# playHing/Scaled-MMD-GAN

Measured on AMD Instinct MI355X. Metric: images/sec/step (64x64 SMMD, batch 64) + MMD-kernel GB/s at 1/2/4/8 GPU, higher is better.
Workload: dtype fp32; 1 GPU; imagenet_smmd 64x64 SNResNet G/D, rbf kernel, scaling, SN, batch 64/GPU, 5D+1G schedule; model=snresnet, global_batch=64, parallelism=dp1, dp_mode=global, dp_forced=False, memory_format=nchw, miopen_winograd=True, miopen_find=False, step_graphs=False, conv_mean_pool=folded 4x4 stride-2 conv, miopen_db=/tmp/code/home/pair/home_parent/tmp/smmd_miopen_db_fofa0w5q

## Files before the change

scaled-mmd-gan_amd/csrc/smmd_wino_s2_wgrad.hip:

```cpp
#include "smmd_wino_common.hpp"

namespace smmd {

namespace {

constexpr int W2_T = 512;
struct for_wino4x4s2_wgrad {};

template <int CT, int RT>
struct S2w {
    static constexpr int NI = 16 / (CT * RT);
    static constexpr int TPI = CT * RT;
    static constexpr int XR = 4 * RT + 2;
    static constexpr int XRS = 4 * CT + 2;
    static constexpr int XS = ((NI * XR * XRS + 3) & ~7) + 4;
    static constexpr int GRS = 2 * CT;
    static constexpr int GS = (NI * 2 * RT * 2 * CT) | 1;
    static constexpr int STAGE = 16 * XS + 64 * GS;
    static constexpr size_t LDS = 2 * STAGE * sizeof(float);
    static constexpr int XF4 = 16 * NI * XR * CT;
    static constexpr int GF4 = 64 * NI * (TPI);
    static constexpr int NX = (XF4 + W2_T - 1) / W2_T;
    static constexpr int NG = (GF4 + W2_T - 1) / W2_T;
    static_assert(CT * RT * NI == 16, "16 tiles per chunk");
    static_assert(XS >= NI * XR * XRS && XS % 8 == 4, "x channel stride");
    static_assert(XRS % 4 == 2, "x row stride");
    static_assert(LDS >= 4 * 9 * 8 * 64 * sizeof(float), "epilogue hand-off fits");
    static_assert(LDS <= 160 * 1024, "LDS budget");
};

struct S2wGeom {
    int N, C, K, H, W;
    int TH, TW, Timg;
    int64_t T;
    int chunks_per_slice;
};

template <int CT, int RT>
__global__ __launch_bounds__(W2_T, 1) void s2_wgrad_kernel(
    const float *__restrict__ x, const float *__restrict__ gy, float *__restrict__ part,
    S2wGeom g) {
    using P = S2w<CT, RT>;
    extern __shared__ float4 s2w_lds4[];
    float *const lds = reinterpret_cast<float *>(s2w_lds4);

    const int tid = threadIdx.x, lane = tid & 63, w = tid >> 6;
    const int kb = blockIdx.x, cb = blockIdx.y, sl = blockIdx.z;
    const int HW = g.H * g.W, Ho = g.H / 2, Wo = g.W / 2, HWo = Ho * Wo;
    const int64_t nchunks_all = g.T / 16;
    const int64_t ch0 = (int64_t)sl * g.chunks_per_slice;
    const int nchunk = (int)min((int64_t)g.chunks_per_slice, nchunks_all - ch0);
    const int cpi = g.Timg >= 16 ? g.Timg / 16 : 1;

    float4 xr[P::NX], gr[P::NG];
    auto gload = [&](int64_t chunk) {
        int n0, ty0;
        if (P::NI > 1) {
            n0 = (int)(chunk * P::NI);
            ty0 = 0;
        } else {
            const uint32_t ch32 = (uint32_t)chunk;
            n0 = (int)(ch32 / (uint32_t)cpi);
            ty0 = (int)(ch32 - (uint32_t)n0 * (uint32_t)cpi) * RT;
        }
        const uint32_t xrange = (uint32_t)(((P::NI - 1) * g.C + 16) * HW) * 4u;
        const uint32_t grange = (uint32_t)(((P::NI - 1) * g.K + 64) * HWo) * 4u;
        const __amdgpu_buffer_rsrc_t xs = __builtin_amdgcn_make_buffer_rsrc(
            const_cast<float *>(x + ((int64_t)n0 * g.C + cb * 16) * HW), 0, xrange, 0x00020000);
        const __amdgpu_buffer_rsrc_t gs = __builtin_amdgcn_make_buffer_rsrc(
            const_cast<float *>(gy + ((int64_t)n0 * g.K + kb * 64) * HWo), 0, grange, 0x00020000);
#pragma unroll
        for (int i = 0; i < P::NX; ++i) {
            const int idx = min(i * W2_T + tid, P::XF4 - 1);
            const int f = idx % CT, rr = idx / CT;
            const int r = rr % P::XR, ci = rr / P::XR;
            const int c = ci % 16, img = ci / 16;
            const int yy = 4 * ty0 - 1 + r;
            const uint32_t off = (yy >= 0 && yy < g.H)
                                     ? (uint32_t)((img * g.C + c) * HW + yy * g.W + 4 * f) * 4u
                                     : BUF_OOB;
            xr[i] = __builtin_bit_cast(float4, __builtin_amdgcn_raw_buffer_load_b128(xs, off, 0, 0));
        }
#pragma unroll
        for (int i = 0; i < P::NG; ++i) {
            const int idx = min(i * W2_T + tid, P::GF4 - 1);
            const int f = idx % P::TPI, ki = idx / P::TPI;
            const int k = ki % 64, img = ki / 64;
            const uint32_t off =
                (uint32_t)((img * g.K + k) * HWo + (2 * ty0) * Wo + 4 * f) * 4u;
            gr[i] = __builtin_bit_cast(float4, __builtin_amdgcn_raw_buffer_load_b128(gs, off, 0, 0));
        }
    };
    auto lstore = [&](int buf) {
        float *X = lds + buf * P::STAGE;
        float *Gd = X + 16 * P::XS;
#pragma unroll
        for (int i = 0; i < P::NX; ++i) {
            const int idx = min(i * W2_T + tid, P::XF4 - 1);
            const int f = idx % CT, rr = idx / CT;
            const int r = rr % P::XR, ci = rr / P::XR;
            const int c = ci % 16, img = ci / 16;
            float *d = X + c * P::XS + (img * P::XR + r) * P::XRS + 1 + 4 * f;
            d[0] = xr[i].x; d[1] = xr[i].y; d[2] = xr[i].z; d[3] = xr[i].w;
        }
#pragma unroll
        for (int i = 0; i < P::NG; ++i) {
            const int idx = min(i * W2_T + tid, P::GF4 - 1);
            const int f = idx % P::TPI, ki = idx / P::TPI;
            const int k = ki % 64, img = ki / 64;
            float *d = Gd + k * P::GS + img * (4 * P::TPI) + 4 * f;
            d[0] = gr[i].x; d[1] = gr[i].y; d[2] = gr[i].z; d[3] = gr[i].w;
        }
    };

    const int tp = w >> 2, kh = (w >> 1) & 1, ch = w & 1, hl = lane >> 5, l32 = lane & 31;
    const int cp = ch * 32 + l32;
    const int cl = cp >> 2, pi = (cp >> 1) & 1, pj = cp & 1;
    auto lds_read = [&](int buf, int s, float (&d)[9], float (&gv)[4]) {
        const float *X = lds + buf * P::STAGE;
        const float *Gd = X + 16 * P::XS;
        const int tau = 2 * s + hl;
        const int img = tau / P::TPI, loc = tau % P::TPI;
        const int ty = loc / CT, tx = loc % CT;
        const float *xc = X + cl * P::XS + (img * P::XR + 4 * ty + pi) * P::XRS + 4 * tx + pj;
#pragma unroll
        for (int a = 0; a < 3; ++a)
#pragma unroll
            for (int b = 0; b < 3; ++b) d[a * 3 + b] = xc[(2 * a) * P::XRS + 2 * b];
        const float *gk = Gd + (kh * 32 + l32) * P::GS + img * (4 * P::TPI) + (2 * ty) * P::GRS +
                          2 * tx;
        gv[0] = gk[0]; gv[1] = gk[1]; gv[2] = gk[P::GRS]; gv[3] = gk[P::GRS + 1];
    };
    auto tslice = [&](int q, const float (&d)[9], const float (&gv)[4], float (&t)[9],
                      float (&a)[9], float (&b)[9]) {
        if (q == 1) {
            const float r0[2] = {gv[0], gv[1]};
            const float r1[2] = {gv[0] + gv[2], gv[1] + gv[3]};
            const float r2[2] = {gv[2], gv[3]};
            a[0] = r0[0]; a[1] = r0[0] + r0[1]; a[2] = r0[1];
            a[3] = r1[0]; a[4] = r1[0] + r1[1]; a[5] = r1[1];
            a[6] = r2[0]; a[7] = r2[0] + r2[1]; a[8] = r2[1];
        } else if (q == 2) {
#pragma unroll
            for (int j = 0; j < 3; ++j) {
                t[j] = d[j] - d[3 + j];
                t[3 + j] = d[3 + j];
                t[6 + j] = d[6 + j] - d[3 + j];
            }
        } else if (q == 3) {
#pragma unroll
            for (int i = 0; i < 3; ++i) {
                b[i * 3 + 0] = t[i * 3 + 0] - t[i * 3 + 1];
                b[i * 3 + 1] = t[i * 3 + 1];
                b[i * 3 + 2] = t[i * 3 + 2] - t[i * 3 + 1];
            }
        }
    };

    f32x16 acc[9];
#pragma unroll
    for (int p = 0; p < 9; ++p) acc[p] = f32x16{};

    for (int i = tid; i < 2 * 16 * P::NI * P::XR; i += W2_T) {
        const int buf = i / (16 * P::NI * P::XR), rc = i % (16 * P::NI * P::XR);
        const int c = rc / (P::NI * P::XR), row = rc % (P::NI * P::XR);
        float *X = lds + buf * P::STAGE + c * P::XS + row * P::XRS;
        X[0] = 0.f;
        X[4 * CT + 1] = 0.f;
    }
    if (nchunk > 0) {
        gload(ch0);
        lstore(0);
        __syncthreads();
        float oa[2][9], ob[2][9];
        {
            float d[9], gv[4], t[9];
            lds_read(0, tp, d, gv);
#pragma unroll
            for (int q = 0; q < 9; ++q) tslice(q, d, gv, t, oa[0], ob[0]);
        }
        for (int c = 0; c < nchunk; ++c) {
            const int buf = c & 1;
            gload(ch0 + min(c + 1, nchunk - 1));
#pragma unroll
            for (int m = 0; m < 4; ++m) {
                const int cur = m & 1, nxt = cur ^ 1;
                float d[9], gv[4], t[9];
                if (m == 3) {
                    lstore(buf ^ 1);
                    __syncthreads();
                }
                __builtin_amdgcn_sched_barrier(0);
                lds_read(m < 3 ? buf : buf ^ 1, m < 3 ? 2 * (m + 1) + tp : tp, d, gv);
                __builtin_amdgcn_sched_barrier(0);
#pragma unroll
                for (int q = 0; q < 9; ++q) {
                    acc[q] = __builtin_amdgcn_mfma_f32_32x32x2f32(oa[cur][q], ob[cur][q], acc[q],
                                                                  0, 0, 0);
                    tslice(q, d, gv, t, oa[nxt], ob[nxt]);
                    __builtin_amdgcn_sched_barrier(0);
                }
            }
        }
    }

    __syncthreads();
    float *out = part + (int64_t)sl * g.K * g.C * 16;
    const int c = cb * 16 + cl;
    float *E = lds + (w & 3) * (9 * 8 * 64);
#pragma unroll
    for (int rh = 0; rh < 2; ++rh) {
        if (tp == 1) {
#pragma unroll
            for (int p = 0; p < 9; ++p)
#pragma unroll
                for (int rr = 0; rr < 8; ++rr) E[(p * 8 + rr) * 64 + lane] = acc[p][rh * 8 + rr];
        }
        __syncthreads();
        if (tp == 0) {
#pragma unroll
            for (int rr = 0; rr < 8; ++rr) {
                const int r = rh * 8 + rr;
                const int k = kb * 64 + kh * 32 + (r & 3) + 8 * (r >> 2) + 4 * hl;
                float u[9];
#pragma unroll
                for (int p = 0; p < 9; ++p) u[p] = acc[p][r] + E[(p * 8 + rr) * 64 + lane];
                float tt[2][3];
#pragma unroll
                for (int j = 0; j < 3; ++j) {
                    tt[0][j] = u[j] + u[3 + j];
                    tt[1][j] = u[3 + j] + u[6 + j];
                }
                float *o = out + ((int64_t)k * g.C + c) * 16;
#pragma unroll
                for (int a = 0; a < 2; ++a) {
                    o[(2 * a + pi) * 4 + pj] = tt[a][0] + tt[a][1];
                    o[(2 * a + pi) * 4 + 2 + pj] = tt[a][1] + tt[a][2];
                }
            }
        }
        __syncthreads();
    }
}

int s2w_shape(int TH, int TW, int *rt) {
    if (TW == 16) { *rt = 1; return 16; }
    if (TW == 8 && TH % 2 == 0) { *rt = 2; return 8; }
    if (TW == 4 && TH % 4 == 0) { *rt = 4; return 4; }
    if (TW == 2 && TH == 2) { *rt = 2; return 2; }
    return 0;
}

template <int CT, int RT>
smmd_status s2w_launch(const float *x, const float *gy, float *part, const S2wGeom &g, int S,
                       hipStream_t st) {
    static bool attr = false;
    if (!attr) {
        if (hipFuncSetAttribute(reinterpret_cast<const void *>(s2_wgrad_kernel<CT, RT>),
                                hipFuncAttributeMaxDynamicSharedMemorySize,
                                (int)S2w<CT, RT>::LDS) != hipSuccess)
            return SMMD_EHIP;
        attr = true;
    }
    s2_wgrad_kernel<CT, RT><<<dim3((unsigned)(g.K / 64), (unsigned)(g.C / 16), (unsigned)S),
                              dim3(W2_T), S2w<CT, RT>::LDS, st>>>(x, gy, part, g);
    return last_launch_status();
}

}

}

using namespace smmd;

extern "C" int smmd_wino4x4s2_wgrad_supported(int n, int ci, int co, int h, int w_img) {
    int rt = 0;
    return n > 0 && ci > 0 && co > 0 && ci % 16 == 0 && co % 64 == 0 && h > 0 && w_img > 0 &&
           h % 4 == 0 && w_img % 4 == 0 && s2w_shape(h / 4, w_img / 4, &rt) != 0 &&
           (int64_t)n * (h / 4) * (w_img / 4) % 16 == 0 &&
           (int64_t)4 * ci * h * w_img * 4 < (1ll << 31) &&
           (int64_t)4 * co * h * w_img < (1ll << 31) && (int64_t)n * (ci + co) * h * w_img < (1ll << 40);
}

extern "C" size_t smmd_wino4x4s2_wgrad_workspace_bytes(int n, int ci, int co, int h, int w_img) {
    if (!smmd_wino4x4s2_wgrad_supported(n, ci, co, h, w_img)) return 0;
    const int64_t T = (int64_t)n * (h / 4) * (w_img / 4);
    const int S = slab_slices((co / 64) * (ci / 16), T / 16, 4);
    return (size_t)(S + slab_groups(S)) * co * ci * 16 * sizeof(float);
}

static smmd_status s2w_launch_all(const float *x, const float *gy, float *gw, int n, int ci,
                                  int co, int h, int w_img, void *ws, size_t ws_bytes, int acc,
                                  smmd_stream_t stream) {
    if (n < 0 || ci <= 0 || co <= 0 || h < 0 || w_img < 0 || !gw) return SMMD_EINVAL;
    hipStream_t st = reinterpret_cast<hipStream_t>(stream);
    if (n == 0 || h == 0 || w_img == 0)
        return acc ? SMMD_OK
                   : hip_status(hipMemsetAsync(gw, 0, (size_t)co * ci * 16 * sizeof(float), st));
    if (!x || !gy) return SMMD_EINVAL;
    if (!smmd_wino4x4s2_wgrad_supported(n, ci, co, h, w_img)) return SMMD_EUNSUPPORTED;
    if ((reinterpret_cast<uintptr_t>(x) | reinterpret_cast<uintptr_t>(gy) |
         reinterpret_cast<uintptr_t>(gw)) & 15)
        return SMMD_EINVAL;
    if (!ws || ws_bytes < smmd_wino4x4s2_wgrad_workspace_bytes(n, ci, co, h, w_img))
        return SMMD_EWORKSPACE;
    if (reinterpret_cast<uintptr_t>(ws) & 15) return SMMD_EINVAL;
    S2wGeom g{};
    g.N = n; g.C = ci; g.K = co; g.H = h; g.W = w_img;
    g.TH = h / 4; g.TW = w_img / 4;
    g.Timg = g.TH * g.TW;
    g.T = (int64_t)n * g.Timg;
    int rt = 0;
    const int ct = s2w_shape(g.TH, g.TW, &rt);
    const int blocks = (co / 64) * (ci / 16);
    const int64_t nchunks = g.T / 16;
    const int S = slab_slices(blocks, nchunks, 4);
    g.chunks_per_slice = (int)((nchunks + S - 1) / S);
    const int Sused = (int)((nchunks + g.chunks_per_slice - 1) / g.chunks_per_slice);
    float *part = static_cast<float *>(ws);
    smmd_status e = ct == 16 ? s2w_launch<16, 1>(x, gy, part, g, Sused, st)
                    : ct == 8 ? s2w_launch<8, 2>(x, gy, part, g, Sused, st)
                    : ct == 4 ? s2w_launch<4, 4>(x, gy, part, g, Sused, st)
                              : s2w_launch<2, 2>(x, gy, part, g, Sused, st);
    if (e != SMMD_OK) return e;
    return slab_sum<for_wino4x4s2_wgrad>(part, Sused, S, (int64_t)co * ci * 4, gw, acc, st);
}

extern "C" smmd_status smmd_wino4x4s2_wgrad(const float *x, const float *gy, float *gw, int n,
                                            int ci, int co, int h, int w_img, void *ws,
                                            size_t ws_bytes, smmd_stream_t stream) {
    return s2w_launch_all(x, gy, gw, n, ci, co, h, w_img, ws, ws_bytes, 0, stream);
}

extern "C" smmd_status smmd_wino4x4s2_wgrad_acc(const float *x, const float *gy, float *gw,
                                                int n, int ci, int co, int h, int w_img,
                                                void *ws, size_t ws_bytes,
                                                smmd_stream_t stream) {
    return s2w_launch_all(x, gy, gw, n, ci, co, h, w_img, ws, ws_bytes, 1, stream);
}
```

Before: 6733 images/s.

## Widen s2 Winograd wgrad block to 32 channels with row-split wave groups

The stride-2 Winograd weight-gradient kernel now covers 32 input channels per block instead of 16. The eight waves are split into two groups that each handle half of the transformed rows (5 or 4 products instead of 9), and the two halves are combined in the epilogue through LDS. Global-to-LDS staging is split into two halves spread across an 8-step inner loop to overlap loads with MFMA, and gy is stored and read as 8-byte pairs. The aim is more reuse of each gy tile per block, fewer redundant transform ops, and better load/compute overlap, at the cost of a larger LDS footprint and half as many blocks along the channel dimension.

```diff
diff --git a/scaled-mmd-gan_amd/csrc/smmd_wino_s2_wgrad.hip b/scaled-mmd-gan_amd/csrc/smmd_wino_s2_wgrad.hip
--- a/scaled-mmd-gan_amd/csrc/smmd_wino_s2_wgrad.hip
+++ b/scaled-mmd-gan_amd/csrc/smmd_wino_s2_wgrad.hip
@@ -15,17 +15,20 @@
     static constexpr int XRS = 4 * CT + 2;
     static constexpr int XS = ((NI * XR * XRS + 3) & ~7) + 4;
     static constexpr int GRS = 2 * CT;
-    static constexpr int GS = (NI * 2 * RT * 2 * CT) | 1;
-    static constexpr int STAGE = 16 * XS + 64 * GS;
+    static constexpr int GS = NI * 2 * RT * 2 * CT + 2;
+    static constexpr int STAGE = 32 * XS + 64 * GS;
     static constexpr size_t LDS = 2 * STAGE * sizeof(float);
-    static constexpr int XF4 = 16 * NI * XR * CT;
-    static constexpr int GF4 = 64 * NI * (TPI);
-    static constexpr int NX = (XF4 + W2_T - 1) / W2_T;
-    static constexpr int NG = (GF4 + W2_T - 1) / W2_T;
-    static_assert(CT * RT * NI == 16, "16 tiles per chunk");
+    static constexpr int XQ = NI * XR * CT;
+    static constexpr int GQ = NI * TPI;
+    static constexpr int NX = (XQ + 15) / 16;
+    static constexpr int NG = GQ / 8;
+    static constexpr int NP = NX + NG;
+    static constexpr int NH = (NP + 1) / 2;
+    static_assert(CT * RT * NI == 16 && 16 % CT == 0 && GQ % 8 == 0, "16 tiles per chunk");
     static_assert(XS >= NI * XR * XRS && XS % 8 == 4, "x channel stride");
     static_assert(XRS % 4 == 2, "x row stride");
-    static_assert(LDS >= 4 * 9 * 8 * 64 * sizeof(float), "epilogue hand-off fits");
+    static_assert(GS % 4 == 2 && GRS % 2 == 0 && STAGE % 2 == 0, "gy pairs 8-byte aligned");
+    static_assert(LDS >= 4 * 2 * 3 * 16 * 64 * sizeof(float), "epilogue hand-off fits");
     static_assert(LDS <= 160 * 1024, "LDS budget");
 };
 
@@ -36,24 +39,29 @@
     int chunks_per_slice;
 };
 
-template <int CT, int RT>
-__global__ __launch_bounds__(W2_T, 1) void s2_wgrad_kernel(
-    const float *__restrict__ x, const float *__restrict__ gy, float *__restrict__ part,
-    S2wGeom g) {
+template <int CT, int RT, int PG>
+__device__ __forceinline__ void s2w_group(const float *__restrict__ x,
+                                          const float *__restrict__ gy,
+                                          float *__restrict__ part, const S2wGeom &g,
+                                          float *const lds, const int cq) {
     using P = S2w<CT, RT>;
-    extern __shared__ float4 s2w_lds4[];
-    float *const lds = reinterpret_cast<float *>(s2w_lds4);
-
-    const int tid = threadIdx.x, lane = tid & 63, w = tid >> 6;
+    constexpr int NPT = PG == 0 ? 5 : 4;
+    const int tid = threadIdx.x, lane = tid & 63;
     const int kb = blockIdx.x, cb = blockIdx.y, sl = blockIdx.z;
     const int HW = g.H * g.W, Ho = g.H / 2, Wo = g.W / 2, HWo = Ho * Wo;
     const int64_t nchunks_all = g.T / 16;
     const int64_t ch0 = (int64_t)sl * g.chunks_per_slice;
     const int nchunk = (int)min((int64_t)g.chunks_per_slice, nchunks_all - ch0);
     const int cpi = g.Timg >= 16 ? g.Timg / 16 : 1;
-
-    float4 xr[P::NX], gr[P::NG];
-    auto gload = [&](int64_t chunk) {
+    const int cw = min(32, g.C - cb * 32);
+
+    const int xc = tid >> 4, xj = tid & 15, gk = tid >> 3, gj = tid & 7;
+    float4 st[P::NP];
+    auto xrow = [&](int i) {
+        const int row = (16 / CT) * i + xj / CT;
+        return 16 * (i + 1) > P::XQ ? min(row, P::NI * P::XR - 1) : row;
+    };
+    auto stage_load = [&](int p0, int p1, int64_t chunk) {
         int n0, ty0;
         if (P::NI > 1) {
             n0 = (int)(chunk * P::NI);
@@ -63,184 +71,200 @@
             n0 = (int)(ch32 / (uint32_t)cpi);
             ty0 = (int)(ch32 - (uint32_t)n0 * (uint32_t)cpi) * RT;
         }
-        const uint32_t xrange = (uint32_t)(((P::NI - 1) * g.C + 16) * HW) * 4u;
+        const uint32_t xrange = (uint32_t)(((P::NI - 1) * g.C + cw) * HW) * 4u;
         const uint32_t grange = (uint32_t)(((P::NI - 1) * g.K + 64) * HWo) * 4u;
         const __amdgpu_buffer_rsrc_t xs = __builtin_amdgcn_make_buffer_rsrc(
-            const_cast<float *>(x + ((int64_t)n0 * g.C + cb * 16) * HW), 0, xrange, 0x00020000);
+            const_cast<float *>(x + ((int64_t)n0 * g.C + cb * 32) * HW), 0, xrange, 0x00020000);
         const __amdgpu_buffer_rsrc_t gs = __builtin_amdgcn_make_buffer_rsrc(
             const_cast<float *>(gy + ((int64_t)n0 * g.K + kb * 64) * HWo), 0, grange, 0x00020000);
 #pragma unroll
         for (int i = 0; i < P::NX; ++i) {
-            const int idx = min(i * W2_T + tid, P::XF4 - 1);
-            const int f = idx % CT, rr = idx / CT;
-            const int r = rr % P::XR, ci = rr / P::XR;
-            const int c = ci % 16, img = ci / 16;
+            if (i < p0 || i >= p1) continue;
+            const int row = xrow(i), f = xj % CT;
+            const int img = P::NI > 1 ? row / P::XR : 0, r = row - img * P::XR;
             const int yy = 4 * ty0 - 1 + r;
             const uint32_t off = (yy >= 0 && yy < g.H)
-                                     ? (uint32_t)((img * g.C + c) * HW + yy * g.W + 4 * f) * 4u
+                                     ? (uint32_t)((img * g.C + xc) * HW + yy * g.W + 4 * f) * 4u
                                      : BUF_OOB;
-            xr[i] = __builtin_bit_cast(float4, __builtin_amdgcn_raw_buffer_load_b128(xs, off, 0, 0));
+            st[i] = __builtin_bit_cast(float4, __builtin_amdgcn_raw_buffer_load_b128(xs, off, 0, 0));
         }
 #pragma unroll
         for (int i = 0; i < P::NG; ++i) {
-            const int idx = min(i * W2_T + tid, P::GF4 - 1);
-            const int f = idx % P::TPI, ki = idx / P::TPI;
-            const int k = ki % 64, img = ki / 64;
+            if (P::NX + i < p0 || P::NX + i >= p1) continue;
+            const int q = gj + 8 * i;
+            const int img = q / P::TPI, f = q % P::TPI;
             const uint32_t off =
-                (uint32_t)((img * g.K + k) * HWo + (2 * ty0) * Wo + 4 * f) * 4u;
-            gr[i] = __builtin_bit_cast(float4, __builtin_amdgcn_raw_buffer_load_b128(gs, off, 0, 0));
-        }
-    };
-    auto lstore = [&](int buf) {
+                (uint32_t)((img * g.K + gk) * HWo + (2 * ty0) * Wo + 4 * f) * 4u;
+            st[P::NX + i] =
+                __builtin_bit_cast(float4, __builtin_amdgcn_raw_buffer_load_b128(gs, off, 0, 0));
+        }
+    };
+    auto stage_store = [&](int p0, int p1, int buf) {
         float *X = lds + buf * P::STAGE;
-        float *Gd = X + 16 * P::XS;
+        float *Gd = X + 32 * P::XS;
 #pragma unroll
         for (int i = 0; i < P::NX; ++i) {
-            const int idx = min(i * W2_T + tid, P::XF4 - 1);
-            const int f = idx % CT, rr = idx / CT;
-            const int r = rr % P::XR, ci = rr / P::XR;
-            const int c = ci % 16, img = ci / 16;
-            float *d = X + c * P::XS + (img * P::XR + r) * P::XRS + 1 + 4 * f;
-            d[0] = xr[i].x; d[1] = xr[i].y; d[2] = xr[i].z; d[3] = xr[i].w;
+            if (i < p0 || i >= p1) continue;
+            float *d = X + xc * P::XS + xrow(i) * P::XRS + 1 + 4 * (xj % CT);
+            d[0] = st[i].x; d[1] = st[i].y; d[2] = st[i].z; d[3] = st[i].w;
         }
 #pragma unroll
         for (int i = 0; i < P::NG; ++i) {
-            const int idx = min(i * W2_T + tid, P::GF4 - 1);
-            const int f = idx % P::TPI, ki = idx / P::TPI;
-            const int k = ki % 64, img = ki / 64;
-            float *d = Gd + k * P::GS + img * (4 * P::TPI) + 4 * f;
-            d[0] = gr[i].x; d[1] = gr[i].y; d[2] = gr[i].z; d[3] = gr[i].w;
-        }
-    };
-
-    const int tp = w >> 2, kh = (w >> 1) & 1, ch = w & 1, hl = lane >> 5, l32 = lane & 31;
-    const int cp = ch * 32 + l32;
+            if (P::NX + i < p0 || P::NX + i >= p1) continue;
+            f2v *d = reinterpret_cast<f2v *>(Gd + gk * P::GS + 4 * (gj + 8 * i));
+            d[0] = f2v{st[P::NX + i].x, st[P::NX + i].y};
+            d[1] = f2v{st[P::NX + i].z, st[P::NX + i].w};
+        }
+    };
+
+    const int hl = lane >> 5, l32 = lane & 31;
+    const int cp = cq * 32 + l32;
     const int cl = cp >> 2, pi = (cp >> 1) & 1, pj = cp & 1;
-    auto lds_read = [&](int buf, int s, float (&d)[9], float (&gv)[4]) {
-        const float *X = lds + buf * P::STAGE;
-        const float *Gd = X + 16 * P::XS;
-        const int tau = 2 * s + hl;
-        const int img = tau / P::TPI, loc = tau % P::TPI;
+    const int xlane = cl * P::XS + (pi + 2 * PG) * P::XRS + pj + 4 * hl;
+    const int glane = 32 * P::XS + l32 * P::GS + 2 * hl;
+    auto lds_read = [&](int buf, int s, float (&d)[6], f2v (&gq)[2][2]) {
+        const int img = (2 * s) / P::TPI, loc = (2 * s) % P::TPI;
         const int ty = loc / CT, tx = loc % CT;
-        const float *xc = X + cl * P::XS + (img * P::XR + 4 * ty + pi) * P::XRS + 4 * tx + pj;
-#pragma unroll
-        for (int a = 0; a < 3; ++a)
-#pragma unroll
-            for (int b = 0; b < 3; ++b) d[a * 3 + b] = xc[(2 * a) * P::XRS + 2 * b];
-        const float *gk = Gd + (kh * 32 + l32) * P::GS + img * (4 * P::TPI) + (2 * ty) * P::GRS +
-                          2 * tx;
-        gv[0] = gk[0]; gv[1] = gk[1]; gv[2] = gk[P::GRS]; gv[3] = gk[P::GRS + 1];
-    };
-    auto tslice = [&](int q, const float (&d)[9], const float (&gv)[4], float (&t)[9],
-                      float (&a)[9], float (&b)[9]) {
-        if (q == 1) {
-            const float r0[2] = {gv[0], gv[1]};
-            const float r1[2] = {gv[0] + gv[2], gv[1] + gv[3]};
-            const float r2[2] = {gv[2], gv[3]};
-            a[0] = r0[0]; a[1] = r0[0] + r0[1]; a[2] = r0[1];
-            a[3] = r1[0]; a[4] = r1[0] + r1[1]; a[5] = r1[1];
-            a[6] = r2[0]; a[7] = r2[0] + r2[1]; a[8] = r2[1];
-        } else if (q == 2) {
-#pragma unroll
-            for (int j = 0; j < 3; ++j) {
-                t[j] = d[j] - d[3 + j];
-                t[3 + j] = d[3 + j];
-                t[6 + j] = d[6 + j] - d[3 + j];
+        const float *xp = lds + buf * P::STAGE + xlane + (img * P::XR + 4 * ty) * P::XRS + 4 * tx;
+#pragma unroll
+        for (int a = 0; a < 2; ++a)
+#pragma unroll
+            for (int b = 0; b < 3; ++b) d[a * 3 + b] = xp[(2 * a) * P::XRS + 2 * b];
+        const float *gp =
+            lds + buf * P::STAGE + glane + img * (4 * P::TPI) + (2 * ty) * P::GRS + 2 * tx;
+#pragma unroll
+        for (int kh = 0; kh < 2; ++kh) {
+            gq[kh][0] = *reinterpret_cast<const f2v *>(gp + kh * 32 * P::GS);
+            gq[kh][1] = *reinterpret_cast<const f2v *>(gp + kh * 32 * P::GS + P::GRS);
+        }
+    };
+    auto form = [&](int q, const float (&d)[6], const f2v (&gq)[2][2], float (&t)[3],
+                    float (&a)[2][5], float (&b)[5]) {
+        if (q == 1 || q == 2) {
+            const int kh = q - 1;
+            const f2v y0 = gq[kh][0], y1 = gq[kh][1];
+            if (PG == 0) {
+                const f2v s = y0 + y1;
+                a[kh][0] = y0.x; a[kh][1] = y0.x + y0.y; a[kh][2] = y0.y;
+                a[kh][3] = s.x; a[kh][4] = s.x + s.y;
+            } else {
+                a[kh][0] = y0.y + y1.y;
+                a[kh][1] = y1.x; a[kh][2] = y1.x + y1.y; a[kh][3] = y1.y;
             }
         } else if (q == 3) {
 #pragma unroll
-            for (int i = 0; i < 3; ++i) {
-                b[i * 3 + 0] = t[i * 3 + 0] - t[i * 3 + 1];
-                b[i * 3 + 1] = t[i * 3 + 1];
-                b[i * 3 + 2] = t[i * 3 + 2] - t[i * 3 + 1];
-            }
-        }
-    };
-
-    f32x16 acc[9];
-#pragma unroll
-    for (int p = 0; p < 9; ++p) acc[p] = f32x16{};
-
-    for (int i = tid; i < 2 * 16 * P::NI * P::XR; i += W2_T) {
-        const int buf = i / (16 * P::NI * P::XR), rc = i % (16 * P::NI * P::XR);
+            for (int j = 0; j < 3; ++j) t[j] = PG == 0 ? d[j] - d[3 + j] : d[3 + j] - d[j];
+        } else if (q == 4) {
+            if (PG == 0) {
+                b[0] = t[0] - t[1]; b[1] = t[1]; b[2] = t[2] - t[1];
+                b[3] = d[3] - d[4]; b[4] = d[4];
+            } else {
+                b[0] = d[2] - d[1];
+                b[1] = t[0] - t[1]; b[2] = t[1]; b[3] = t[2] - t[1];
+            }
+        }
+    };
+
+    f32x16 acc[2][NPT];
+#pragma unroll
+    for (int p = 0; p < 2 * NPT; ++p) acc[p & 1][p >> 1] = f32x16{};
+
+    for (int i = tid; i < 2 * 32 * P::NI * P::XR; i += W2_T) {
+        const int buf = i / (32 * P::NI * P::XR), rc = i % (32 * P::NI * P::XR);
         const int c = rc / (P::NI * P::XR), row = rc % (P::NI * P::XR);
         float *X = lds + buf * P::STAGE + c * P::XS + row * P::XRS;
         X[0] = 0.f;
         X[4 * CT + 1] = 0.f;
     }
     if (nchunk > 0) {
-        gload(ch0);
-        lstore(0);
+        stage_load(0, P::NP, ch0);
+        stage_store(0, P::NP, 0);
         __syncthreads();
-        float oa[2][9], ob[2][9];
+        float oa[2][2][5], ob[2][5];
+        auto kstep = [&](int cur, int rbuf, int rs) {
+            const int nxt = cur ^ 1;
+            float d[6], t[3];
+            f2v gq[2][2];
+            __builtin_amdgcn_sched_barrier(0);
+            lds_read(rbuf, rs, d, gq);
+            __builtin_amdgcn_sched_barrier(0);
+#pragma unroll
+            for (int q = 0; q < 2 * NPT; ++q) {
+                const int p = q >> 1, kh = q & 1;
+                acc[kh][p] = __builtin_amdgcn_mfma_f32_32x32x2f32(oa[cur][kh][p], ob[cur][p],
+                                                                  acc[kh][p], 0, 0, 0);
+                form(q, d, gq, t, oa[nxt], ob[nxt]);
+                __builtin_amdgcn_sched_barrier(0);
+            }
+        };
         {
-            float d[9], gv[4], t[9];
-            lds_read(0, tp, d, gv);
-#pragma unroll
-            for (int q = 0; q < 9; ++q) tslice(q, d, gv, t, oa[0], ob[0]);
+            float d[6], t[3];
+            f2v gq[2][2];
+            lds_read(0, 0, d, gq);
+#pragma unroll
+            for (int q = 1; q < 5; ++q) form(q, d, gq, t, oa[0], ob[0]);
         }
         for (int c = 0; c < nchunk; ++c) {
             const int buf = c & 1;
-            gload(ch0 + min(c + 1, nchunk - 1));
-#pragma unroll
-            for (int m = 0; m < 4; ++m) {
-                const int cur = m & 1, nxt = cur ^ 1;
-                float d[9], gv[4], t[9];
+            const int64_t nc = ch0 + min(c + 1, nchunk - 1);
+#pragma unroll
+            for (int m = 0; m < 8; ++m) {
+                if (m == 0) stage_load(0, P::NH, nc);
                 if (m == 3) {
-                    lstore(buf ^ 1);
-                    __syncthreads();
+                    stage_store(0, P::NH, buf ^ 1);
+                    stage_load(P::NH, P::NP, nc);
                 }
-                __builtin_amdgcn_sched_barrier(0);
-                lds_read(m < 3 ? buf : buf ^ 1, m < 3 ? 2 * (m + 1) + tp : tp, d, gv);
-                __builtin_amdgcn_sched_barrier(0);
-#pragma unroll
-                for (int q = 0; q < 9; ++q) {
-                    acc[q] = __builtin_amdgcn_mfma_f32_32x32x2f32(oa[cur][q], ob[cur][q], acc[q],
-                                                                  0, 0, 0);
-                    tslice(q, d, gv, t, oa[nxt], ob[nxt]);
-                    __builtin_amdgcn_sched_barrier(0);
-                }
+                if (m == 6) stage_store(P::NH, P::NP, buf ^ 1);
+                if (m == 7) __syncthreads();
+                const int rbuf = m < 7 ? buf : buf ^ 1, rs = m < 7 ? m + 1 : 0;
+                kstep(m & 1, rbuf, rs);
             }
         }
     }
 
     __syncthreads();
     float *out = part + (int64_t)sl * g.K * g.C * 16;
-    const int c = cb * 16 + cl;
-    float *E = lds + (w & 3) * (9 * 8 * 64);
-#pragma unroll
-    for (int rh = 0; rh < 2; ++rh) {
-        if (tp == 1) {
-#pragma unroll
-            for (int p = 0; p < 9; ++p)
-#pragma unroll
-                for (int rr = 0; rr < 8; ++rr) E[(p * 8 + rr) * 64 + lane] = acc[p][rh * 8 + rr];
-        }
-        __syncthreads();
-        if (tp == 0) {
-#pragma unroll
-            for (int rr = 0; rr < 8; ++rr) {
-                const int r = rh * 8 + rr;
+    const int c = cb * 32 + cl;
+    float *E = lds + cq * (2 * 3 * 16 * 64);
+    if (PG == 1) {
+#pragma unroll
+        for (int kh = 0; kh < 2; ++kh)
+#pragma unroll
+            for (int r = 0; r < 16; ++r) {
+                float *e = E + (kh * 3 * 16 + r) * 64 + lane;
+                e[0] = acc[kh][0][r];
+                e[16 * 64] = acc[kh][1][r] + acc[kh][2][r];
+                e[2 * 16 * 64] = (acc[kh][0][r] + acc[kh][2][r]) + acc[kh][NPT - 1][r];
+            }
+    }
+    __syncthreads();
+    if (PG == 0 && c < g.C) {
+#pragma unroll
+        for (int kh = 0; kh < 2; ++kh)
+#pragma unroll
+            for (int r = 0; r < 16; ++r) {
                 const int k = kb * 64 + kh * 32 + (r & 3) + 8 * (r >> 2) + 4 * hl;
-                float u[9];
-#pragma unroll
-                for (int p = 0; p < 9; ++p) u[p] = acc[p][r] + E[(p * 8 + rr) * 64 + lane];
-                float tt[2][3];
-#pragma unroll
-                for (int j = 0; j < 3; ++j) {
-                    tt[0][j] = u[j] + u[3 + j];
-                    tt[1][j] = u[3 + j] + u[6 + j];
-                }
+                const float *e = E + (kh * 3 * 16 + r) * 64 + lane;
+                const float u00 = acc[kh][0][r], u01 = acc[kh][1][r], u02 = acc[kh][2][r];
+                const float u10 = acc[kh][3][r], u11 = acc[kh][NPT - 1][r];
                 float *o = out + ((int64_t)k * g.C + c) * 16;
-#pragma unroll
-                for (int a = 0; a < 2; ++a) {
-                    o[(2 * a + pi) * 4 + pj] = tt[a][0] + tt[a][1];
-                    o[(2 * a + pi) * 4 + 2 + pj] = tt[a][1] + tt[a][2];
-                }
-            }
-        }
-        __syncthreads();
-    }
+                o[pi * 4 + pj] = (u00 + u01) + (u10 + u11);
+                o[pi * 4 + 2 + pj] = ((u01 + u02) + u11) + e[0];
+                o[(2 + pi) * 4 + pj] = (u10 + u11) + e[16 * 64];
+                o[(2 + pi) * 4 + 2 + pj] = u11 + e[2 * 16 * 64];
+            }
+    }
+}
+
+template <int CT, int RT>
+__global__ __launch_bounds__(W2_T, 1) void s2_wgrad_kernel(
+    const float *__restrict__ x, const float *__restrict__ gy, float *__restrict__ part,
+    S2wGeom g) {
+    extern __shared__ float4 s2w_lds4[];
+    float *const lds = reinterpret_cast<float *>(s2w_lds4);
+    const int w = __builtin_amdgcn_readfirstlane(threadIdx.x >> 6);
+    if (w < 4) s2w_group<CT, RT, 0>(x, gy, part, g, lds, w);
+    else s2w_group<CT, RT, 1>(x, gy, part, g, lds, w - 4);
 }
 
 int s2w_shape(int TH, int TW, int *rt) {
@@ -262,7 +286,7 @@
             return SMMD_EHIP;
         attr = true;
     }
-    s2_wgrad_kernel<CT, RT><<<dim3((unsigned)(g.K / 64), (unsigned)(g.C / 16), (unsigned)S),
+    s2_wgrad_kernel<CT, RT><<<dim3((unsigned)(g.K / 64), (unsigned)((g.C + 31) / 32), (unsigned)S),
                               dim3(W2_T), S2w<CT, RT>::LDS, st>>>(x, gy, part, g);
     return last_launch_status();
 }
@@ -285,7 +309,7 @@
 extern "C" size_t smmd_wino4x4s2_wgrad_workspace_bytes(int n, int ci, int co, int h, int w_img) {
     if (!smmd_wino4x4s2_wgrad_supported(n, ci, co, h, w_img)) return 0;
     const int64_t T = (int64_t)n * (h / 4) * (w_img / 4);
-    const int S = slab_slices((co / 64) * (ci / 16), T / 16, 4);
+    const int S = slab_slices((co / 64) * ((ci + 31) / 32), T / 16, 4);
     return (size_t)(S + slab_groups(S)) * co * ci * 16 * sizeof(float);
 }
 
@@ -312,7 +336,7 @@
     g.T = (int64_t)n * g.Timg;
     int rt = 0;
     const int ct = s2w_shape(g.TH, g.TW, &rt);
-    const int blocks = (co / 64) * (ci / 16);
+    const int blocks = (co / 64) * ((ci + 31) / 32);
     const int64_t nchunks = g.T / 16;
     const int S = slab_slices(blocks, nchunks, 4);
     g.chunks_per_slice = (int)((nchunks + S - 1) / S);
```

After: 6795 images/s (median of 6 runs). No clear change (+0.9%).
